# christophmark/bayesloop

Measured on AMD Instinct MI355X. Metric: grid-cells*timesteps/sec (fit()), higher is better.
Workload: dtype f64; 1 GPU; C4 HyperStudy 512x512 grid x 512 sigma values, T=256, full fit (forward+backward+average posterior); T=256, n_hyper=512, mode=full, parallelism=hyper-grid points dealt round-robin to 1 GPU(s), one RCCL gather + one reduce

## Files before the change

bayesloop_amd/csrc/blhip_chainres.hpp:

```cpp
#pragma once
#include "blhip_mfma.hpp"
#include "blhip_resident.hpp"

namespace blc {

using blf::exp_mn;
using blf::reflect1;
using blf::sldi;
using blf::DMAX;
using blk::NRED;
using blm::d4;

constexpr int NT = 512, NW = 8;
constexpr int TM = 16;
constexpr int WCOL = 16;
constexpr int NSLOT = 8;
constexpr int MAXLAG = 4;
constexpr int MAX_STRIPS = 64;
constexpr int SCALE_WAVE = 6;

struct ChainParams {
    int n0, n1, strips;
    int n0t, n1t;
    int T, d, rec_len, lag;
// ... 133 lines not shown
    Q.n0t = own_sgpr(P.n0t);
    Q.n1t = own_sgpr(P.n1t);
    Q.T = own_sgpr(P.T);
    Q.d = own_sgpr(P.d);
    Q.rec_len = own_sgpr(P.rec_len);
    Q.lag = own_sgpr(P.lag);
    Q.means = own_sgpr(P.means);
    Q.strip_major = own_sgpr(P.strip_major);
    Q.B = own_sgpr(P.B);
    Q.nslots = own_sgpr(P.nslots);
    Q.nblk = own_sgpr(P.nblk);
    Q.chain_ids = own_sgpr(P.chain_ids);
    Q.tap_id = own_sgpr(P.tap_id);
    Q.taps = own_sgpr(P.taps);
    Q.tap_off = own_sgpr(P.tap_off);
    Q.tap_lw = own_sgpr(P.tap_lw);
    Q.src0 = own_sgpr(P.src0);
    Q.kinds = own_sgpr(P.kinds);
    Q.reset = own_sgpr(P.reset);
    Q.post = own_sgpr(P.post);
    Q.post_stride = own_sgpr(P.post_stride);
    Q.m0 = own_sgpr(P.m0);
    Q.m1 = own_sgpr(P.m1);
    Q.colA = own_sgpr(P.colA);
    Q.colB = own_sgpr(P.colB);
    Q.rec = own_sgpr(P.rec);
    Q.step0 = own_sgpr(P.step0);
    Q.psum = own_sgpr(P.psum);
    Q.gran = own_sgpr(P.gran);
    Q.sfwd = own_sgpr(P.sfwd);
    Q.wchain = own_sgpr(P.wchain);
    Q.infirst = own_sgpr(P.infirst);
    Q.part = own_sgpr(P.part);
    Q.part_stride = own_sgpr(P.part_stride);
    Q.zeros = own_sgpr(P.zeros);
    Q.part_fresh = own_sgpr(P.part_fresh);
    Q.tshare = own_sgpr(P.tshare);
    Q.bprov = own_sgpr(P.bprov);
    Q.skip_prefix = own_sgpr(P.skip_prefix);
    Q.abort_word = own_sgpr(P.abort_word);
    Q.timeout_ticks = own_sgpr(P.timeout_ticks);
    Q.prof = own_sgpr(P.prof);
    Q.lik = own_sgpr(P.lik);
    Q.tap_id1 = own_sgpr(P.tap_id1);
    Q.xch = own_sgpr(P.xch);
    Q.xch_chain = own_sgpr(P.xch_chain);
    Q.lik_nat = own_sgpr(P.lik_nat);
    Q.xch_mode = own_sgpr(P.xch_mode);
    Q.anch = own_sgpr(P.anch);
    return Q;
}

__device__ __forceinline__ double ldnt(const double *base, unsigned byteoff) { return __builtin_nontemporal_load((const double *)((const char *)base + byteoff)); }
__device__ __forceinline__ void stnt(double *base, unsigned byteoff, double v) { __builtin_nontemporal_store(v, (double *)((char *)base + byteoff)); }

__device__ __forceinline__ double nan_if(bool nan, double x) {
    return __hiloint2double(nan ? 0x7ff80000 : __double2hiint(x), __double2loint(x));
}

#ifndef BLC_BAND4
#define BLC_BAND4 1
#endif
#ifndef BLC_FASTEDGE
#define BLC_FASTEDGE 1
#endif
#ifndef BLC_HOIST_A
#define BLC_HOIST_A 1
#endif
#ifndef BLC_OWNREG
#define BLC_OWNREG 1
#endif
#ifndef BLC_CIRC_RING
#define BLC_CIRC_RING 1
#endif
#ifndef BLC_HOIST_LOOP
#define BLC_HOIST_LOOP 1
#endif
#ifndef BLC_FOLD_HOIST_MAX
#define BLC_FOLD_HOIST_MAX 20
#endif
#ifndef BLC_FOLD4_HOIST_MAX
#define BLC_FOLD4_HOIST_MAX 14
#endif
typedef const double __attribute__((address_space(3))) *band_cp;
template <int NK, int OFF = 0, int NR = NK, int AST = 64>
__device__ __forceinline__ d4 band_products(band_cp Al, const double (&Bv)[NR]) {
    static_assert(OFF + NK <= NR, "the tile's window lies inside the ring");
#if BLC_BAND4
    double a0 = 0.0, a1 = 0.0, a2 = 0.0, a3 = 0.0;
#pragma unroll
    for (int s = 0; s < NK - 3; ++s) {
        const double A = Al[s * AST];
        a0 = __builtin_amdgcn_mfma_f64_4x4x4f64(A, Bv[OFF + s], a0, 0, 0, 0);
        a1 = __builtin_amdgcn_mfma_f64_4x4x4f64(A, Bv[OFF + s + 1], a1, 0, 0, 0);
        a2 = __builtin_amdgcn_mfma_f64_4x4x4f64(A, Bv[OFF + s + 2], a2, 0, 0, 0);
        a3 = __builtin_amdgcn_mfma_f64_4x4x4f64(A, Bv[OFF + s + 3], a3, 0, 0, 0);
    }
    return d4{a0, a1, a2, a3};
#else
    static_assert(AST == 64, "the 16x16x4 form: one entry per lane");
    d4 acc = {0.0, 0.0, 0.0, 0.0};
#pragma unroll
    for (int kb = 0; kb < NK; ++kb) acc = __builtin_amdgcn_mfma_f64_16x16x4f64(Al[kb * 64], Bv[OFF + kb], acc, 0, 0, 0);
    return acc;
#endif
}
template <int NK, int OFF = 0, int NR = NK>
__device__ __forceinline__ d4 band_products_w(const double (&Aw)[NK > 3 ? NK - 3 : 1], const double (&Bv)[NR]) {
    static_assert(OFF + NK <= NR, "the tile's window lies inside the ring");
    double a0 = 0.0, a1 = 0.0, a2 = 0.0, a3 = 0.0;
#pragma unroll
    for (int s = 0; s < NK - 3; ++s) {
        a0 = __builtin_amdgcn_mfma_f64_4x4x4f64(Aw[s], Bv[OFF + s], a0, 0, 0, 0);
        a1 = __builtin_amdgcn_mfma_f64_4x4x4f64(Aw[s], Bv[OFF + s + 1], a1, 0, 0, 0);
        a2 = __builtin_amdgcn_mfma_f64_4x4x4f64(Aw[s], Bv[OFF + s + 2], a2, 0, 0, 0);
        a3 = __builtin_amdgcn_mfma_f64_4x4x4f64(Aw[s], Bv[OFF + s + 3], a3, 0, 0, 0);
    }
    return d4{a0, a1, a2, a3};
}
template <int NK> constexpr int ring_mod() { return NK % 4 == 0 ? NK : NK + 2; }
template <int NK, int NR>
__device__ __forceinline__ d4 band_products_wc(const double (&Aw)[NK > 3 ? NK - 3 : 1], const double (&Bv)[NR], int first) {
    double a0 = 0.0, a1 = 0.0, a2 = 0.0, a3 = 0.0;
#pragma unroll
    for (int s = 0; s < NK - 3; ++s) {
        a0 = __builtin_amdgcn_mfma_f64_4x4x4f64(Aw[s], Bv[(first + s) % NR], a0, 0, 0, 0);
        a1 = __builtin_amdgcn_mfma_f64_4x4x4f64(Aw[s], Bv[(first + s + 1) % NR], a1, 0, 0, 0);
        a2 = __builtin_amdgcn_mfma_f64_4x4x4f64(Aw[s], Bv[(first + s + 2) % NR], a2, 0, 0, 0);
        a3 = __builtin_amdgcn_mfma_f64_4x4x4f64(Aw[s], Bv[(first + s + 3) % NR], a3, 0, 0, 0);
    }
    return d4{a0, a1, a2, a3};
}
template <int NK, int NR, int AST>
__device__ __forceinline__ d4 band_products_c(band_cp Al, const double (&Bv)[NR], int first) {
    double a0 = 0.0, a1 = 0.0, a2 = 0.0, a3 = 0.0;
#pragma unroll
    for (int s = 0; s < NK - 3; ++s) {
        const double A = Al[s * AST];
        a0 = __builtin_amdgcn_mfma_f64_4x4x4f64(A, Bv[(first + s) % NR], a0, 0, 0, 0);
        a1 = __builtin_amdgcn_mfma_f64_4x4x4f64(A, Bv[(first + s + 1) % NR], a1, 0, 0, 0);
        a2 = __builtin_amdgcn_mfma_f64_4x4x4f64(A, Bv[(first + s + 2) % NR], a2, 0, 0, 0);
        a3 = __builtin_amdgcn_mfma_f64_4x4x4f64(A, Bv[(first + s + 3) % NR], a3, 0, 0, 0);
    }
    return d4{a0, a1, a2, a3};
}
__device__ __forceinline__ int band_distance(int e, int R0) {
#if BLC_BAND4
    return abs(4 * (e >> 6) + ((e & 63) >> 4) - R0 - (e & 3));
#else
    return abs(4 * (e >> 6) + ((e & 63) >> 4) - R0 - (e & 15));
#endif
}
__device__ __forceinline__ int band_distance16(int e, int R0) { return abs(4 * (e >> 4) + ((e & 15) >> 2) - R0 - (e & 3)); }


template <int NR>
__device__ __forceinline__ void ring_fill_first_wave(double (&Bv)[NR], const double *S, int g, int c, int k0, int cnt, int rel0) {
    const double *sm = S + (3 - g) * WCOL + c;
    const double *s0 = S + g * WCOL + c;
#pragma unroll
    for (int q = 0; q < NR; ++q) {
        const int rel = rel0 + 4 * q;
        if (q < cnt) Bv[k0 + q] = rel < 0 ? sm[(-rel - 4) * WCOL] : s0[rel * WCOL];
    }
}
template <int N0, int ROWS_W, int NR>
__device__ __forceinline__ void ring_fill_last_wave(double (&Bv)[NR], const double *S, int g, int c, int k0, int cnt, int rel0, int kmod = 0) {
    constexpr int row0 = N0 - ROWS_W;
    const int relmax = rel0 + 4 * (cnt - 1);
    const double *sm = S + (2 * N0 - 1 - row0 - relmax - g) * WCOL + c;
    const double *s0 = S + (row0 + rel0 + g) * WCOL + c;
#pragma unroll
    for (int q = 0; q < NR; ++q) {
        const int rel = rel0 + 4 * q;
        if (q < cnt) Bv[kmod ? (k0 + q) % kmod : k0 + q] = rel >= ROWS_W ? sm[(relmax - rel) * WCOL] : s0[(rel - rel0) * WCOL];
    }
}

template <int NK, int NTW>
constexpr size_t lds_doubles() { return (size_t)(NTW > 4 ? 1 : 2) * NW * NTW * TM * WCOL + NK * (NTW > 4 ? 16 : 64) + NW * NTW * TM + 2 * NW * 4 * 5 + 2 * NSLOT + 8; }

#ifdef BLC_PROF
#define BLC_STAMP(i) do { if (prof_me && k >= 8 && k < 24) P.prof[(wv ? 256 : 0) + (k - 8) * 16 + (i)] = __builtin_readcyclecounter(); } while (0)
#else
#define BLC_STAMP(i) do { } while (0)
#endif

template <int NK, int NTW, bool BWD, bool STORE, bool PAD = false, bool TAB = false>
__global__ __launch_bounds__(NT, 1) void chain_kernel(const ChainParams P) {
    static_assert(!TAB || NTW <= 4, "tabulated likelihood: geometries of <= 512 rows");
    constexpr int R0 = (4 * NK - TM) / 2;
    constexpr int N0 = NW * NTW * TM;
    constexpr int XSZ = N0 * WCOL;
    static_assert(!(PAD && BWD && !STORE) || NTW > 4, "padded grids of <= 512 rows: the folding backward pass is chain_fold2_kernel's");
    static_assert(!(PAD && BWD && STORE && NTW > 4), "padded grids of 1024 rows: posteriors are folded, never stored");
    const int n0t = PAD ? P.n0t : N0, n1t = PAD ? P.n1t : P.n1;
    static_assert(NK == 4 || (NK >= 6 && R0 % 4 == 0), "band = 16 + 2 R0 columns, R0 a multiple of 4; NK = 4: no stencil");
    constexpr bool FILTER = NK > 4;
    constexpr bool TALL = NTW > 4;
    extern __shared__ __attribute__((aligned(16))) double lds[];
    double *const X = lds;
    constexpr int AST = (TALL && BLC_BAND4) ? 16 : 64;
    double *const As = X + (TALL ? 1 : 2) * XSZ;
    double *const m0s = As + NK * AST;
    double *const red = m0s + N0;
    double *const scal = red + 2 * NW * 4 * 5;
    double *const iscal = scal + NSLOT;

    const int tid = threadIdx.x, lane = tid & 63;
    const int wv = __builtin_amdgcn_readfirstlane(tid >> 6);
    const int cs = blockIdx.x / P.strips, tj = blockIdx.x - cs * P.strips;
    const int b = sldi(P.chain_ids, cs);
    const int tap = sldi(P.tap_id, b);
    const int lw0 = tap >= 0 ? sldi(P.tap_lw, tap) : 0;
    const long long o0 = tap >= 0 ? sldi(P.tap_off, tap) : 0;
    const int gj = tj * WCOL + (lane & 15);
    const long long G = (long long)P.n0 * P.n1;
    const int tsh = (!FILTER && P.tshare) ? sldi(P.tshare, b) : 0;

    if (FILTER) for (int e = tid; e < NK * AST; e += NT) As[e] = (AST == 16 ? band_distance16(e, R0) : band_distance(e, R0)) == 0 ? 1.0 : 0.0;
    for (int e = tid; e < N0; e += NT) m0s[e] = P.m0[PAD ? min(e, n0t - 1) : e];
// ... 360 lines not shown
#pragma unroll
                for (int r = 0; r < 4; ++r)
                    al[it % ALD][r] = (it + ALD < NTW) ? ldnt(pstep, cell_off(l, it + ALD, r)) : ldnt(pnext, cell_off(l, it + ALD - NTW, r));
            }
            if ((BWD || STORE) && P.means) {
#pragma unroll
                for (int r = 0; r < 4; ++r) { sM0 = fma(acc[r], m0s[i + g + 4 * r], sM0); sM1 = fma(acc[r], g1, sM1); }
            }

            if (it == 0) BLC_STAMP(4);
            if (it == NTW - 1) BLC_STAMP(5);
            if (FILTER && !WHOLE_RING && it + 1 < NTW) {
#pragma unroll
                for (int kb = 0; kb < NK - 4; ++kb) Bv[kb] = Bv[kb + 4];
                if (FASTEDGE && wv == NW - 1 && (it + 1) * TM + R0 + 12 >= NTW * TM) ring_fill_last_wave<N0, NTW * TM>(Bv, S, g, c, NK - 4, 4, (it + 1) * TM + R0);
                else if (!FASTEDGE && edge) {
#pragma unroll
                    for (int q = 0; q < 4; ++q) Bv[NK - 4 + q] = S[reflect1(i + TM + R0 + 4 * q + g, n0t) * WCOL + c];
                } else {
                    const double *s1 = S + (i + TM + R0 + g) * WCOL + c;
#pragma unroll
                    for (int q = 0; q < 4; ++q) Bv[NK - 4 + q] = s1[q * 4 * WCOL];
                }
            }
        }

        double v[5] = {sN, sS, BWD ? sC : sM0, BWD ? sM0 : sM1, sM1};
        constexpr int NV = BWD ? 5 : 4;
        const int nv = BWD ? (P.means ? 5 : 3) : (P.means ? 4 : ((!FILTER && P.kinds) ? 2 : 1));
        double *rk = red + (k & 1) * (NW * 4 * 5);
#pragma unroll
        for (int q = 0; q < NV; ++q) {
            if (q < nv) {
                double x = v[q];
                x = blk::dpp_add<0x111, 0xf>(x);
                x = blk::dpp_add<0x112, 0xf>(x);
                x = blk::dpp_add<0x114, 0xf>(x);
                x = blk::dpp_add<0x118, 0xf>(x);
                if ((lane & 15) == 15) rk[(wv * 4 + (lane >> 4)) * 5 + q] = x;
            }
        }
        BLC_STAMP(6);
        __syncthreads();
        BLC_STAMP(7);
        if (TALL && FILTER) {
            const int l = fresh_lane(), g = l >> 4, c = l & 15;
#pragma unroll
            for (int it = 0; it < NTW; ++it)
#pragma unroll
                for (int r = 0; r < 4; ++r) D[(row0 + it * TM + g + 4 * r) * WCOL + c] = nst[it][r];
        }
        if (FILTER && k == 0) {
            for (int e = tid; e < NK * AST; e += NT) {
                const int a = AST == 16 ? band_distance16(e, R0) : band_distance(e, R0);
                As[e] = a == 0 ? (lw0 > 0 ? P.taps[o0] : 1.0) : (a <= lw0 ? P.taps[o0 + a] : 0.0);
            }
        }
        if (FILTER && (TALL || k == 0)) __syncthreads();
        if (wv == 5 && lane < nv) {
            double tot = 0.0;
#pragma unroll
            for (int w = 0; w < NW * 4; ++w) tot += rk[w * 5 + lane];
            const int slot = BWD ? lane : (lane < 2 ? lane : lane + 1);
            if (lane == 0 || (BWD ? (P.means || lane < 3) : (lane == 1 ? (!FILTER && P.kinds != nullptr) : P.means != 0)))
                P.psum[(((long long)t * P.B + b) * NRED + slot) * P.nblk + tj] = tot;
            if (lane == (BWD ? 2 : 0)) {
                const unsigned long long bits = (unsigned long long)__double_as_longlong(tot);
                const unsigned long long tag = (unsigned long long)(unsigned)(k + 1) << 32;
                unsigned long long *gw = P.gran + ((((long long)(k & (NSLOT - 1)) * P.nslots + cs) * P.strips + tj) << 1);
                blr::st_u64(gw, tag | (bits & 0xffffffffull));
                blr::st_u64(gw + 1, tag | (bits >> 32));
            }
        }
#pragma unroll
        for (int q = 0; q < DMAX; ++q) xd[q] = xn[q];
        if constexpr (ANCT) anc = anc_next;
    }
}


template <int NK, int NTW>
constexpr size_t lds_doubles_fold2() { return (size_t)2 * NW * NTW * TM * WCOL + 2 * NK * (NK > 24 ? 16 : 64) + NW * NTW * TM + 2 * 2 * NW * 4 * 3 + 4 * NSLOT + 8; }

template <int NK, int NTW>
constexpr size_t lds_doubles_fold4() { return (size_t)2 * NW * NTW * TM * WCOL + 2 * NK * 64 + 4 * 2 * NW * 4 * 3 + 8 * NSLOT + 8; }

template <int NK, int NTW>
__device__ __forceinline__ void chain_fold4_body(const ChainParams &P) {
    static_assert(NK >= 6 && NK <= 24 && NTW >= 1 && NTW <= 4, "four chains per block: ring lengths 6 .. 24 on <= 512 rows");
    constexpr int R0 = (4 * NK - TM) / 2;
    static_assert(R0 % 4 == 0, "band = 16 + 2 R0 columns, R0 a multiple of 4");
    constexpr int N0 = NW * NTW * TM;
    constexpr int XSZ = N0 * WCOL;
    constexpr int AST = 64;
    constexpr int HC = WCOL / 2;
    constexpr unsigned ROWB = HC * 8u, ROW4B = 4u * ROWB;
    extern __shared__ __attribute__((aligned(16))) double lds[];
    double *const X = lds;
    double *const As = X + 2 * XSZ;
    double *const red = As + 2 * NK * AST;
    double *const scal = red + 4 * 2 * NW * 4 * 3;
    double *const iscal = scal + 4 * NSLOT;

    const int tid = threadIdx.x, lane = tid & 63;
    const int wv = __builtin_amdgcn_readfirstlane(tid >> 6);
    const int cs4 = blockIdx.x / P.strips, tj = blockIdx.x - cs4 * P.strips;
    const int nch = min(4, P.nslots - 4 * cs4);
    const int npair = (nch + 1) >> 1;
    int bch[4], lw0[4];
    long long o0[4];
#pragma unroll
    for (int q = 0; q < 4; ++q) {
        bch[q] = sldi(P.chain_ids, 4 * cs4 + min(q, nch - 1));
        const int tap = sldi(P.tap_id, bch[q]);
        lw0[q] = tap >= 0 ? sldi(P.tap_lw, tap) : 0;
        o0[q] = tap >= 0 ? sldi(P.tap_off, tap) : 0;
    }
    const int hl = (lane >> 3) & 1;
    const long long G = (long long)P.n0 * P.n1;

    for (int e = tid; e < 2 * NK * AST; e += NT) As[e] = band_distance(e % (NK * AST), R0) == 0 ? 1.0 : 0.0;
    if (tid < 8 * NSLOT) scal[tid] = 1.0;
    for (int e = tid; e < 2 * XSZ; e += NT) {
        const int q = e % XSZ, row = q >> 4, col = tj * HC + (q & 7);
        X[e] = P.src0[(long long)row * P.n1 + col];
    }
    const double cA = P.colA[tj * HC + (lane & 7)];
    const unsigned strip0 = (unsigned)tj * (unsigned)(P.n0 * HC * 8);
    const int row0 = wv * (NTW * TM);
    auto fresh_lane = [&]() { int l = lane; asm volatile("" : "+v"(l)); return l; };
    auto cell_off = [&](int l, int it) { return __umul24(row0 + it * TM + (l >> 4), ROWB) + strip0 + (unsigned)(l & 7) * 8u; };

    const int t_first = P.T - 1;
    double *const pslot = P.part + (long long)cs4 * P.part_stride;
    int slot_l[2];
    const double *post_l[2], *sfwd_l[2];
    double wch[2], inpred[2];
#pragma unroll
    for (int j = 0; j < 2; ++j) {
        const int q = 2 * j + hl;
        const int b = hl ? bch[2 * j + 1] : bch[2 * j];
        slot_l[j] = min(q, nch - 1) * NSLOT;
        post_l[j] = P.post + (long long)b * P.post_stride;
        sfwd_l[j] = P.sfwd + (long long)b * P.T;
        wch[j] = q < nch ? P.wchain[b] : 0.0;
        inpred[j] = P.infirst[b];
    }
    double stt[NTW][4], al[NTW][4], pacc[NTW][4];
    {
        const double *p0 = post_l[0] + (long long)t_first * G;
        const double *a0 = pslot + (long long)t_first * G;
#pragma unroll
        for (int it = 0; it < NTW; ++it)
#pragma unroll
            for (int r = 0; r < 4; ++r) {
                const unsigned off = cell_off(lane, it) + r * ROW4B;
                al[it][r] = blm::ld32(p0, off);
                pacc[it][r] = (P.part_fresh || (r >> 1) != hl) ? blm::ld32(P.zeros, off & 4088u) : blm::ld32(a0, off);
                stt[it][r] = 0.0;
            }
    }
    double sf_next = 1.0;
    if (wv == SCALE_WAVE || wv == 5 || wv == 0 || wv == NW - 1) __builtin_amdgcn_s_setprio(2);
    bool dead = false;
    typedef const double __attribute__((address_space(3))) *lds_cp;
    unsigned long long gq0[4] = {0ull, 0ull, 0ull, 0ull}, gq1[4] = {0ull, 0ull, 0ull, 0ull};
    double Sprev[4] = {1.0, 1.0, 1.0, 1.0};
    double mq = 1.0, iq = 1.0, dn_prev = -1.0;
    int nq = 0;
    double a_mE = 1.0, a_mR = 1.0, a_iE = 1.0, a_iR = 1.0;
    int a_nE = 0, a_nR = 0;
    const int astrips = P.strips >> 1, atj = tj >> 1;
    auto anchor_lane = [&](int l) { return (l & 0x30) | ((tj & 1) << 3) | (l & 7); };
    AnchorEntry anc_next = anchor_load(P.anch, t_first, wv, astrips, atj, anchor_lane(lane));
    int pend_j = -1, pend_k = 0;

    const LoopParams Q = loop_params(P);
    auto totals = [&](int j, int k) {
        const int hh = (lane >> 3) & 1, q = lane & 7, c = 2 * j + hh;
        if (wv == 5 && lane < 16 && q < 3 && c < nch) {
            const double *rk = red + (c * 2 + (k & 1)) * (NW * 4 * 3);
            double tot = 0.0;
#pragma unroll
            for (int w = 0; w < NW * 4; ++w) tot += rk[w * 3 + q];
            const int t = Q.T - 1 - k;
            const int b = hh ? (j ? bch[3] : bch[1]) : (j ? bch[2] : bch[0]);
            Q.psum[(((long long)t * Q.B + b) * NRED + q) * Q.nblk + tj] = tot;
            if (q == 2) {
                const unsigned long long bits = (unsigned long long)__double_as_longlong(tot);
                const unsigned long long tag = (unsigned long long)(unsigned)(k + 1) << 32;
                unsigned long long *gw = Q.gran + ((((long long)(k & (NSLOT - 1)) * Q.nslots + 4 * cs4 + c) * Q.strips + tj) << 1);
                blr::st_u64(gw, tag | (bits & 0xffffffffull));
                blr::st_u64(gw + 1, tag | (bits >> 32));
            }
        }
    };
    __syncthreads();

    const bool scale_wave = wv == SCALE_WAVE;
    const int nsteps = Q.T * npair;
#pragma unroll 1
    for (int cstep = 0; cstep < nsteps; ++cstep) {
        const int k = npair == 2 ? cstep >> 1 : cstep;
        const int j = __builtin_amdgcn_readfirstlane(npair == 2 ? cstep & 1 : 0);
        const int t = Q.T - 1 - k;
        const int tn = (k + 1 < Q.T) ? t - 1 : t;
        const int jn = k + 1;
        double *const pslot_t = pslot + (long long)t * G;
        double *const pslot_tn = pslot + (long long)tn * G;
        double *const Xj = X + j * XSZ;
        const bool need = scale_wave && jn >= Q.lag && jn < Q.T;
        const bool mine = need && lane < Q.strips;
        unsigned long long hq0[2], hq1[2];
#pragma unroll
        for (int hh = 0; hh < 2; ++hh) {
            hq0[hh] = j ? gq0[2 + hh] : gq0[hh]; hq1[hh] = j ? gq1[2 + hh] : gq1[hh];
            if (scale_wave && 2 * j + hh < nch && jn + 1 >= Q.lag && jn + 1 < Q.T && lane < Q.strips) {
                const unsigned long long *gn = Q.gran + ((((long long)((jn + 1 - Q.lag) & (NSLOT - 1)) * Q.nslots + 4 * cs4 + 2 * j + hh) * Q.strips + lane) << 1);
                const unsigned long long n0_ = blr::ld_u64(gn), n1_ = blr::ld_u64(gn + 1);
                if (j) { gq0[2 + hh] = n0_; gq1[2 + hh] = n1_; } else { gq0[hh] = n0_; gq1[hh] = n1_; }
            }
        }
        const bool last_pair = j + 1 == npair;
        const int tnext = last_pair ? tn : t;
        const double sf_now = sf_next;
        sf_next = (last_pair ? sfwd_l[0] : sfwd_l[1])[min(tnext + 1, Q.T - 1)];
        __syncthreads();
        if (pend_j >= 0) {
            double *const Xp = X + pend_j * XSZ;
            const int l = fresh_lane(), g = l >> 4, c = l & 15;
#pragma unroll
            for (int it = 0; it < NTW; ++it)
#pragma unroll
                for (int r = 0; r < 4; ++r) Xp[(row0 + it * TM + g + 4 * r) * WCOL + c] = stt[it][r];
            totals(pend_j, pend_k);
        }
        if (npair == 1 && pend_j >= 0) __syncthreads();
        pend_j = j; pend_k = k;

        constexpr bool FASTEDGE = BLC_FASTEDGE && NTW * TM >= R0;
        const bool edge = row0 < R0 || row0 + NTW * TM + R0 > N0;
        constexpr int NRM = BLC_CIRC_RING ? ring_mod<NK>() : NK;
        double Bv[NRM];
        {
            const int l = fresh_lane(), g = l >> 4, c = l & 15;
            if (FASTEDGE && wv == 0) ring_fill_first_wave(Bv, Xj, g, c, 0, NK, -R0);
            else if (FASTEDGE && wv == NW - 1 && R0 + 12 >= NTW * TM) ring_fill_last_wave<N0, NTW * TM>(Bv, Xj, g, c, 0, NK, -R0);
            else if (!FASTEDGE && edge) {
#pragma unroll
                for (int kb = 0; kb < NK; ++kb) Bv[kb] = Xj[reflect1(row0 - R0 + 4 * kb + g, N0) * WCOL + c];
            } else {
                const double *s0 = Xj + (row0 - R0 + g) * WCOL + c;
#pragma unroll
                for (int kb = 0; kb < NK; ++kb) Bv[kb] = s0[kb * 4 * WCOL];
            }
        }
        double scale = 1.0, wq = 0.0, wfloor = 0.0;
        double mE = 1.0, mR = 1.0, iE = 1.0, iR = 1.0;
        int nE = 0, nR = 0;
        double sN = 0.0, sS = 0.0, sC = 0.0;
        const double *const pnext = (last_pair ? post_l[0] : post_l[1]) + (long long)tnext * G;

        constexpr bool HOISTA = BLC_HOIST_A && BLC_BAND4 && NTW >= 2 && NK <= BLC_FOLD4_HOIST_MAX;
        double Aw[HOISTA ? NK - 3 : 1];
        if constexpr (HOISTA) {
            const int l = fresh_lane();
            const unsigned aoff = (unsigned)l * 8u + (unsigned)(j * NK * AST * 8);
            lds_cp Al = (lds_cp)((const char __attribute__((address_space(3))) *)(lds_cp)As + aoff);
#pragma unroll
            for (int q = 0; q < NK - 3; ++q) Aw[q] = Al[q * AST];
        }
#pragma unroll
        for (int it = 0; it < NTW; ++it) {
            const int i = row0 + it * TM;
            const int l = fresh_lane(), g = l >> 4, c = l & 15;
            const int h = (l >> 3) & 1;
            d4 acc = {0.0, 0.0, 0.0, 0.0};
            if constexpr (HOISTA) {
                acc = band_products_wc<NK, NRM>(Aw, Bv, BLC_CIRC_RING ? 4 * it : 0);
            } else {
                const unsigned aoff = (unsigned)l * 8u + (unsigned)(j * NK * AST * 8);
                lds_cp Al = (lds_cp)((const char __attribute__((address_space(3))) *)(lds_cp)As + aoff);
                acc = band_products_c<NK, NRM, AST>(Al, Bv, BLC_CIRC_RING ? 4 * it : 0);
            }
            if (it == 0) {
                const int sl = (j ? slot_l[1] : slot_l[0]) + (k & (NSLOT - 1));
                scale = scal[sl];
                double ip = j ? inpred[1] : inpred[0];
                if (k > 0) ip = ip * sf_now * iscal[sl];
                if (j) inpred[1] = ip; else inpred[0] = ip;
                const double wc = j ? wch[1] : wch[0];
                wq = wc * ip; wfloor = wc * 1e-300;
                if (scale_wave) {
#pragma unroll
                    for (int hh = 0; hh < 2; ++hh) {
                        const int cq = 2 * j + hh;
                        if (cq < nch) {
                            double sj = 1.0;
                            if (need) {
                                const unsigned long long *gp = Q.gran + ((((long long)((jn - Q.lag) & (NSLOT - 1)) * Q.nslots + 4 * cs4 + cq) * Q.strips + lane) << 1);
                                const unsigned long long want = (unsigned long long)(unsigned)(jn - Q.lag + 1);
                                unsigned long long q0 = hq0[hh], q1 = hq1[hh];
                                bool ok = !mine || ((q0 >> 32) == want && (q1 >> 32) == want);
                                if (!dead && !__all(ok)) {
                                    const unsigned long long t0 = blr::now_ticks();
                                    for (unsigned spins = 1; !__all(ok); ++spins) {
                                        if (!ok) { q0 = blr::ld_u64(gp); q1 = blr::ld_u64(gp + 1); ok = (q0 >> 32) == want && (q1 >> 32) == want; }
                                        blr::nap();
                                        if ((spins & 255u) == 0u) {
                                            if (blr::ld_flag(Q.abort_word) != 0u) { dead = true; break; }
                                            if (blr::now_ticks() - t0 > Q.timeout_ticks) { blr::st_flag(Q.abort_word, 1u); dead = true; break; }
                                        }
                                    }
                                }
                                const double v = mine ? __longlong_as_double((long long)((q0 & 0xffffffffull) | (q1 << 32))) : 0.0;
                                const double Sg = blk::wave_sum(v);
                                const double sp = j ? Sprev[2 + hh] : Sprev[hh];
                                sj = dead ? 1.0 : sp * scal[cq * NSLOT + ((jn - Q.lag) & (NSLOT - 1))] / Sg;
                                if (j) Sprev[2 + hh] = Sg; else Sprev[hh] = Sg;
                            }
                            if (lane == 0) { scal[cq * NSLOT + (jn & (NSLOT - 1))] = sj; iscal[cq * NSLOT + (jn & (NSLOT - 1))] = 1.0 / sj; }
                        }
                    }
                }
                if (j == 0) {
                    anchor_unpack(anc_next, a_mE, a_nE, a_mR, a_nR);
                    const double dn = anc_next.dn;
                    if (dn != dn_prev) {
                        const double d2 = -32.0 * cA * dn * Q.step0 * Q.step0;
                        int tmp;
                        exp_mn(d2, mq, nq);
                        exp_mn(-d2, iq, tmp);
                        dn_prev = dn;
                    }
                    a_iE = blmath::inv_m(a_mE); a_iR = blmath::inv_m(a_mR);
                    anc_next = anchor_load(Q.anch, tn, wv, astrips, atj, anchor_lane(fresh_lane()));
                }
                mE = a_mE; nE = a_nE; mR = a_mR; nR = a_nR; iE = a_iE; iR = a_iR;
            }

#pragma unroll
            for (int r = 0; r < 4; ++r) {
                const double Lv = ldexp(mE, nE);
                const double beta = acc[r] * scale;
                const double p = al[it][r] * beta;
                const double cn = beta * Lv;
                const double pl = nan_if(Lv == 0.0, ldexp(p * iE, -nE));
                stt[it][r] = cn;
                pacc[it][r] += fmax(p * wq, wfloor);
                sN += p; sS += pl; sC += cn;
                mE *= mR; nE += nR;
                mR *= mq; nR += nq;
                iE *= iR; iR *= iq;
            }
            const unsigned off_t = cell_off(l, it);
            if (last_pair) {
                double tot[4];
#pragma unroll
                for (int r = 0; r < 4; ++r) tot[r] = blk::dpp_add<0x128, 0xf>(pacc[it][r]);
                char *const ps = (char *)pslot_t + off_t + (h ? 2u * ROW4B : 0u);
                __builtin_nontemporal_store(h ? tot[2] : tot[0], (double *)ps);
                __builtin_nontemporal_store(h ? tot[3] : tot[1], (double *)(ps + ROW4B));
                const char *const pz = (const char *)Q.zeros + (off_t & 2040u);
                const char *const pn = (const char *)pslot_tn + off_t;
                const char *const p01 = (Q.part_fresh || h) ? pz : pn, *const p23 = (Q.part_fresh || !h) ? pz : pn;
                pacc[it][0] = __builtin_nontemporal_load((const double *)p01);
                pacc[it][1] = __builtin_nontemporal_load((const double *)(p01 + ROW4B));
                pacc[it][2] = __builtin_nontemporal_load((const double *)(p23 + 2 * ROW4B));
                pacc[it][3] = __builtin_nontemporal_load((const double *)(p23 + 3 * ROW4B));
            }
            {
                const char *const pa_ = (const char *)pnext + off_t;
#pragma unroll
                for (int r = 0; r < 4; ++r) al[it][r] = __builtin_nontemporal_load((const double *)(pa_ + r * ROW4B));
            }
            if (it + 1 < NTW) {
                constexpr bool CIRC = BLC_CIRC_RING != 0;
                if (!CIRC) {
#pragma unroll
                    for (int kb = 0; kb < NK - 4; ++kb) Bv[kb] = Bv[kb + 4];
                }
                const int e0 = CIRC ? 4 * it + NK : NK - 4;
                if (FASTEDGE && wv == NW - 1 && (it + 1) * TM + R0 + 12 >= NTW * TM) ring_fill_last_wave<N0, NTW * TM>(Bv, Xj, g, c, e0, 4, (it + 1) * TM + R0, CIRC ? NRM : 0);
                else if (!FASTEDGE && edge) {
#pragma unroll
                    for (int q = 0; q < 4; ++q) Bv[CIRC ? (e0 + q) % NRM : e0 + q] = Xj[reflect1(i + TM + R0 + 4 * q + g, N0) * WCOL + c];
                } else {
                    const double *s1 = Xj + (i + TM + R0 + g) * WCOL + c;
#pragma unroll
                    for (int q = 0; q < 4; ++q) Bv[CIRC ? (e0 + q) % NRM : e0 + q] = s1[q * 4 * WCOL];
                }
            }
        }

        {
            double v[3] = {sN, sS, sC};
            const int l = fresh_lane();
            double *rk = red + ((2 * j + ((l >> 3) & 1)) * 2 + (k & 1)) * (NW * 4 * 3);
#pragma unroll
            for (int q = 0; q < 3; ++q) {
                double x = v[q];
                x = blk::dpp_add<0x111, 0xf>(x);
                x = blk::dpp_add<0x112, 0xf>(x);
                x = blk::dpp_add<0x114, 0xf>(x);
                if ((l & 7) == 7) rk[(wv * 4 + (l >> 4)) * 3 + q] = x;
            }
        }
        if (k == 0 && last_pair) {
            __syncthreads();
            {
                double *const Xp = X + pend_j * XSZ;
                const int l = fresh_lane(), g = l >> 4, c = l & 15;
#pragma unroll
                for (int it = 0; it < NTW; ++it)
#pragma unroll
                    for (int r = 0; r < 4; ++r) Xp[(row0 + it * TM + g + 4 * r) * WCOL + c] = stt[it][r];
                totals(pend_j, pend_k);
                pend_j = -1;
            }
            for (int e = tid; e < 2 * NK * AST; e += NT) {
                const int jj = e / (NK * AST), q = e - jj * (NK * AST);
                const int cq = 2 * jj + ((q >> 3) & 1);
                const int lw = cq == 0 ? lw0[0] : (cq == 1 ? lw0[1] : (cq == 2 ? lw0[2] : lw0[3]));
                const long long o = cq == 0 ? o0[0] : (cq == 1 ? o0[1] : (cq == 2 ? o0[2] : o0[3]));
                const int a = band_distance(q, R0);
                As[e] = a == 0 ? (lw > 0 ? P.taps[o] : 1.0) : (a <= lw ? P.taps[o + a] : 0.0);
            }
        }
    }
    __syncthreads();
    if (pend_j >= 0) totals(pend_j, pend_k);
}

template <int NK, int NTW, bool PAD, bool QUAD>
__global__ __launch_bounds__(NT, 1) void chain_fold2_kernel(const ChainParams P) {
    static_assert(QUAD && !PAD, "the four-argument flavour: four chains per block on an exact geometry");
    chain_fold4_body<NK, NTW>(P);
}

template <int NK, int NTW, bool PAD = false>
__global__ __launch_bounds__(NT, 1) void chain_fold2_kernel(const ChainParams P) {
    constexpr int R0 = (4 * NK - TM) / 2;
    constexpr int N0 = NW * NTW * TM;
    constexpr int XSZ = N0 * WCOL;
    const int n0t = PAD ? P.n0t : N0, n1t = PAD ? P.n1t : P.n1;
    static_assert(NK == 4 || (NK >= 6 && R0 % 4 == 0), "band = 16 + 2 R0 columns, R0 a multiple of 4; NK = 4: no stencil");
    constexpr bool FILTER = NK > 4;
    extern __shared__ __attribute__((aligned(16))) double lds[];
    double *const X = lds;
    constexpr int AST = (NK > 24 && BLC_BAND4) ? 16 : 64;
    double *const As = X + 2 * XSZ;
    double *const m0s = As + 2 * NK * AST;
    double *const red = m0s + N0;
    double *const scal = red + 2 * 2 * NW * 4 * 3;
    double *const iscal = scal + 2 * NSLOT;

    const int tid = threadIdx.x, lane = tid & 63;
    const int wv = __builtin_amdgcn_readfirstlane(tid >> 6);
    const int cs2 = blockIdx.x / P.strips, tj = blockIdx.x - cs2 * P.strips;
    const int nch = min(2, P.nslots - 2 * cs2);
    int bch[2], tap[2], lw0[2], tshv[2];
    long long o0[2];
#pragma unroll
    for (int j = 0; j < 2; ++j) {
        bch[j] = sldi(P.chain_ids, 2 * cs2 + min(j, nch - 1));
        tshv[j] = P.tshare ? sldi(P.tshare, bch[j]) : 0;
        tap[j] = sldi(P.tap_id, bch[j]);
        lw0[j] = tap[j] >= 0 ? sldi(P.tap_lw, tap[j]) : 0;
        o0[j] = tap[j] >= 0 ? sldi(P.tap_off, tap[j]) : 0;
    }
    const int gj = tj * WCOL + (lane & 15);
    const long long G = (long long)P.n0 * P.n1;

    if (FILTER) for (int e = tid; e < 2 * NK * AST; e += NT) As[e] = (AST == 16 ? band_distance16(e % (NK * AST), R0) : band_distance(e % (NK * AST), R0)) == 0 ? 1.0 : 0.0;
    for (int e = tid; e < N0; e += NT) m0s[e] = P.m0[PAD ? min(e, n0t - 1) : e];
    if (tid < 4 * NSLOT) scal[tid] = 1.0;
    for (int e = tid; e < 2 * XSZ; e += NT) {
        const int q = e % XSZ, row = q >> 4, col = tj * WCOL + (q & 15);
        X[e] = (!PAD || (row < n0t && col < n1t)) ? P.src0[(long long)row * n1t + col] : 0.0;
    }
    const bool colok = !PAD || gj < n1t;
    const int gjc = PAD ? min(gj, n1t - 1) : gj;
    const double cA = P.colA[gjc], cB = P.colB[gjc];
    const unsigned rowx8 = (unsigned)WCOL * 8u;
    const unsigned strip0 = (unsigned)tj * (unsigned)(P.n0 * WCOL * 8);
    const int row0 = wv * (NTW * TM);
    auto fresh_lane = [&]() { int l = lane; asm volatile("" : "+v"(l)); return l; };
    auto cell_off = [&](int l, int it, int r) { return __umul24(row0 + it * TM + (l >> 4) + 4 * r, rowx8) + strip0 + (unsigned)(l & 15) * 8u; };

    const int t_first = P.T - 1;
// ... 311 lines not shown
```

Before: 181.1 billion grid-cells*timesteps/s.

## Defer fold4 state writes past MFMA, partially hoist band A, stage scale tags in LDS

In the four-chain fold kernel, the write of the previous pair's state into LDS is moved from before the MFMA band products to just after the first tile's products. This lets the LDS stores overlap matrix work instead of sitting on the critical path after the barrier. Band matrix entries are now partially hoisted into registers for larger ring lengths, using a per-(NK,NTW) table. Granule tags and the previous scale sums move from per-pair registers into LDS to cut register pressure. The cost is more LDS use, more code paths, and a risk that the reordered state writes race with readers if the barrier assumptions don't hold.

```diff
diff --git a/bayesloop_amd/csrc/blhip_chainres.hpp b/bayesloop_amd/csrc/blhip_chainres.hpp
--- a/bayesloop_amd/csrc/blhip_chainres.hpp
+++ b/bayesloop_amd/csrc/blhip_chainres.hpp
@@ -239,6 +239,15 @@
 #ifndef BLC_FOLD4_HOIST_MAX
 #define BLC_FOLD4_HOIST_MAX 14
 #endif
+#ifndef BLC_FOLD4_LATE_WRITES
+#define BLC_FOLD4_LATE_WRITES 1
+#endif
+#ifndef BLC_FOLD4_SCALE_LDS
+#define BLC_FOLD4_SCALE_LDS 1
+#endif
+#ifndef BLC_FOLD4_HOIST_PART
+#define BLC_FOLD4_HOIST_PART 1
+#endif
 typedef const double __attribute__((address_space(3))) *band_cp;
 template <int NK, int OFF = 0, int NR = NK, int AST = 64>
 __device__ __forceinline__ d4 band_products(band_cp Al, const double (&Bv)[NR]) {
@@ -294,6 +303,20 @@
 #pragma unroll
     for (int s = 0; s < NK - 3; ++s) {
         const double A = Al[s * AST];
+        a0 = __builtin_amdgcn_mfma_f64_4x4x4f64(A, Bv[(first + s) % NR], a0, 0, 0, 0);
+        a1 = __builtin_amdgcn_mfma_f64_4x4x4f64(A, Bv[(first + s + 1) % NR], a1, 0, 0, 0);
+        a2 = __builtin_amdgcn_mfma_f64_4x4x4f64(A, Bv[(first + s + 2) % NR], a2, 0, 0, 0);
+        a3 = __builtin_amdgcn_mfma_f64_4x4x4f64(A, Bv[(first + s + 3) % NR], a3, 0, 0, 0);
+    }
+    return d4{a0, a1, a2, a3};
+}
+template <int NK, int NR, int AST, int H>
+__device__ __forceinline__ d4 band_products_hc(const double (&Aw)[H > 0 ? H : 1], band_cp Al, const double (&Bv)[NR], int first) {
+    static_assert(H >= 0 && H <= NK - 3, "hoisted entries: a prefix of the band");
+    double a0 = 0.0, a1 = 0.0, a2 = 0.0, a3 = 0.0;
+#pragma unroll
+    for (int s = 0; s < NK - 3; ++s) {
+        const double A = s < H ? Aw[s < H ? s : 0] : Al[s * AST];
         a0 = __builtin_amdgcn_mfma_f64_4x4x4f64(A, Bv[(first + s) % NR], a0, 0, 0, 0);
         a1 = __builtin_amdgcn_mfma_f64_4x4x4f64(A, Bv[(first + s + 1) % NR], a1, 0, 0, 0);
         a2 = __builtin_amdgcn_mfma_f64_4x4x4f64(A, Bv[(first + s + 2) % NR], a2, 0, 0, 0);
@@ -820,8 +843,20 @@
 template <int NK, int NTW>
 constexpr size_t lds_doubles_fold2() { return (size_t)2 * NW * NTW * TM * WCOL + 2 * NK * (NK > 24 ? 16 : 64) + NW * NTW * TM + 2 * 2 * NW * 4 * 3 + 4 * NSLOT + 8; }
 
+template <int NK> constexpr bool fold4_scale_lds() { return BLC_FOLD4_SCALE_LDS != 0 && NK <= 20; }
+constexpr int FOLD4_GST = 4 * 64 * 2 + 8;
+template <int NK, int NTW> constexpr int fold4_hoist() {
+    if (!(BLC_HOIST_A && BLC_BAND4) || NTW < 2) return 0;
+    if (NK <= BLC_FOLD4_HOIST_MAX) return NK - 3;
+    if (!BLC_FOLD4_HOIST_PART) return 0;
+    if (NTW == 2) return NK - 3;
+    if (NTW == 3) return NK == 24 ? 15 : NK == 22 ? 17 : NK - 3;
+    return NK == 16 ? 10 : NK == 18 ? 11 : NK == 20 ? 9 : NK == 22 ? 3 : 0;
+}
 template <int NK, int NTW>
-constexpr size_t lds_doubles_fold4() { return (size_t)2 * NW * NTW * TM * WCOL + 2 * NK * 64 + 4 * 2 * NW * 4 * 3 + 8 * NSLOT + 8; }
+constexpr size_t lds_doubles_fold4() {
+    return (size_t)2 * NW * NTW * TM * WCOL + 2 * NK * 64 + 4 * 2 * NW * 4 * 3 + 8 * NSLOT + 8 + (fold4_scale_lds<NK>() ? FOLD4_GST : 0);
+}
 
 template <int NK, int NTW>
 __device__ __forceinline__ void chain_fold4_body(const ChainParams &P) {
@@ -833,12 +868,18 @@
     constexpr int AST = 64;
     constexpr int HC = WCOL / 2;
     constexpr unsigned ROWB = HC * 8u, ROW4B = 4u * ROWB;
+    constexpr int LATE = (NK == 24 && NTW == 4) ? 0 : BLC_FOLD4_LATE_WRITES;
+    static_assert(LATE >= 0 && LATE <= 2, "BLC_FOLD4_LATE_WRITES: 0, 1 or 2");
     extern __shared__ __attribute__((aligned(16))) double lds[];
     double *const X = lds;
     double *const As = X + 2 * XSZ;
     double *const red = As + 2 * NK * AST;
     double *const scal = red + 4 * 2 * NW * 4 * 3;
     double *const iscal = scal + 4 * NSLOT;
+    constexpr bool GLDS = fold4_scale_lds<NK>();
+    static_assert(lds_doubles_fold4<NK, NTW>() * sizeof(double) <= 160 * 1024, "four-chain fold kernel: the LDS of a CU");
+    unsigned long long *const gst = (unsigned long long *)(iscal + 4 * NSLOT + 8);
+    double *const sprv = (double *)(gst + 4 * 64 * 2);
 
     const int tid = threadIdx.x, lane = tid & 63;
     const int wv = __builtin_amdgcn_readfirstlane(tid >> 6);
@@ -859,6 +900,10 @@
 
     for (int e = tid; e < 2 * NK * AST; e += NT) As[e] = band_distance(e % (NK * AST), R0) == 0 ? 1.0 : 0.0;
     if (tid < 8 * NSLOT) scal[tid] = 1.0;
+    if constexpr (GLDS) {
+        for (int e = tid; e < 4 * 64 * 2; e += NT) gst[e] = 0ull;
+        if (tid < 4) sprv[tid] = 1.0;
+    }
     for (int e = tid; e < 2 * XSZ; e += NT) {
         const int q = e % XSZ, row = q >> 4, col = tj * HC + (q & 7);
         X[e] = P.src0[(long long)row * P.n1 + col];
@@ -895,9 +940,16 @@
                 const unsigned off = cell_off(lane, it) + r * ROW4B;
                 al[it][r] = blm::ld32(p0, off);
                 pacc[it][r] = (P.part_fresh || (r >> 1) != hl) ? blm::ld32(P.zeros, off & 4088u) : blm::ld32(a0, off);
-                stt[it][r] = 0.0;
-            }
-    }
+                stt[it][r] = LATE ? P.src0[(long long)(row0 + it * TM + (lane >> 4) + 4 * r) * P.n1 + tj * HC + (lane & 7)] : 0.0;
+            }
+    }
+    auto state_out = [&](double *Xp, int it0, int it1) {
+        const int l = fresh_lane(), g = l >> 4, c = l & 15;
+#pragma unroll
+        for (int it = 0; it < NTW; ++it)
+#pragma unroll
+            for (int r = 0; r < 4; ++r) if (it >= it0 && it < it1) Xp[(row0 + it * TM + g + 4 * r) * WCOL + c] = stt[it][r];
+    };
     double sf_next = 1.0;
     if (wv == SCALE_WAVE || wv == 5 || wv == 0 || wv == NW - 1) __builtin_amdgcn_s_setprio(2);
     bool dead = false;
@@ -913,6 +965,15 @@
     AnchorEntry anc_next = anchor_load(P.anch, t_first, wv, astrips, atj, anchor_lane(lane));
     int pend_j = -1, pend_k = 0;
 
+#ifdef BLC_PROF
+#ifndef BLC_PROF_WAVE4
+#define BLC_PROF_WAVE4 2
+#endif
+    const bool prof_me = blockIdx.x == 0 && lane == 0 && (wv == 0 || wv == BLC_PROF_WAVE4);
+#define BLC_STAMP4(i) do { if (prof_me && cstep >= 16 && cstep < 32) P.prof[(wv ? 256 : 0) + (cstep - 16) * 16 + (i)] = __builtin_readcyclecounter(); } while (0)
+#else
+#define BLC_STAMP4(i) do { } while (0)
+#endif
     const LoopParams Q = loop_params(P);
     auto totals = [&](int j, int k) {
         const int hh = (lane >> 3) & 1, q = lane & 7, c = 2 * j + hh;
@@ -944,19 +1005,34 @@
         const int t = Q.T - 1 - k;
         const int tn = (k + 1 < Q.T) ? t - 1 : t;
         const int jn = k + 1;
+        BLC_STAMP4(0);
         double *const pslot_t = pslot + (long long)t * G;
         double *const pslot_tn = pslot + (long long)tn * G;
         double *const Xj = X + j * XSZ;
         const bool need = scale_wave && jn >= Q.lag && jn < Q.T;
         const bool mine = need && lane < Q.strips;
-        unsigned long long hq0[2], hq1[2];
-#pragma unroll
-        for (int hh = 0; hh < 2; ++hh) {
-            hq0[hh] = j ? gq0[2 + hh] : gq0[hh]; hq1[hh] = j ? gq1[2 + hh] : gq1[hh];
-            if (scale_wave && 2 * j + hh < nch && jn + 1 >= Q.lag && jn + 1 < Q.T && lane < Q.strips) {
-                const unsigned long long *gn = Q.gran + ((((long long)((jn + 1 - Q.lag) & (NSLOT - 1)) * Q.nslots + 4 * cs4 + 2 * j + hh) * Q.strips + lane) << 1);
-                const unsigned long long n0_ = blr::ld_u64(gn), n1_ = blr::ld_u64(gn + 1);
-                if (j) { gq0[2 + hh] = n0_; gq1[2 + hh] = n1_; } else { gq0[hh] = n0_; gq1[hh] = n1_; }
+        [[maybe_unused]] unsigned long long hq0[2], hq1[2];
+        if constexpr (GLDS) {
+            if (scale_wave) {
+                unsigned long long *const gs = gst + ((npair == 2 ? 2 * (1 - j) : 0) * 64 + fresh_lane()) * 2;
+#pragma unroll
+                for (int hh = 0; hh < 2; ++hh) { gs[hh * 128] = gq0[hh]; gs[hh * 128 + 1] = gq1[hh]; }
+            }
+#pragma unroll
+            for (int hh = 0; hh < 2; ++hh)
+                if (scale_wave && 2 * j + hh < nch && jn + 1 >= Q.lag && jn + 1 < Q.T && lane < Q.strips) {
+                    const unsigned long long *gn = Q.gran + ((((long long)((jn + 1 - Q.lag) & (NSLOT - 1)) * Q.nslots + 4 * cs4 + 2 * j + hh) * Q.strips + lane) << 1);
+                    gq0[hh] = blr::ld_u64(gn); gq1[hh] = blr::ld_u64(gn + 1);
+                }
+        } else {
+#pragma unroll
+            for (int hh = 0; hh < 2; ++hh) {
+                hq0[hh] = j ? gq0[2 + hh] : gq0[hh]; hq1[hh] = j ? gq1[2 + hh] : gq1[hh];
+                if (scale_wave && 2 * j + hh < nch && jn + 1 >= Q.lag && jn + 1 < Q.T && lane < Q.strips) {
+                    const unsigned long long *gn = Q.gran + ((((long long)((jn + 1 - Q.lag) & (NSLOT - 1)) * Q.nslots + 4 * cs4 + 2 * j + hh) * Q.strips + lane) << 1);
+                    const unsigned long long n0_ = blr::ld_u64(gn), n1_ = blr::ld_u64(gn + 1);
+                    if (j) { gq0[2 + hh] = n0_; gq1[2 + hh] = n1_; } else { gq0[hh] = n0_; gq1[hh] = n1_; }
+                }
             }
         }
         const bool last_pair = j + 1 == npair;
@@ -964,17 +1040,21 @@
         const double sf_now = sf_next;
         sf_next = (last_pair ? sfwd_l[0] : sfwd_l[1])[min(tnext + 1, Q.T - 1)];
         __syncthreads();
+        BLC_STAMP4(1);
         if (pend_j >= 0) {
-            double *const Xp = X + pend_j * XSZ;
-            const int l = fresh_lane(), g = l >> 4, c = l & 15;
-#pragma unroll
-            for (int it = 0; it < NTW; ++it)
-#pragma unroll
-                for (int r = 0; r < 4; ++r) Xp[(row0 + it * TM + g + 4 * r) * WCOL + c] = stt[it][r];
+            if (!LATE || npair == 1) {
+                double *const Xp = X + pend_j * XSZ;
+                const int l = fresh_lane(), g = l >> 4, c = l & 15;
+#pragma unroll
+                for (int it = 0; it < NTW; ++it)
+#pragma unroll
+                    for (int r = 0; r < 4; ++r) Xp[(row0 + it * TM + g + 4 * r) * WCOL + c] = stt[it][r];
+            }
             totals(pend_j, pend_k);
         }
         if (npair == 1 && pend_j >= 0) __syncthreads();
         pend_j = j; pend_k = k;
+        double *const Xo = X + (1 - j) * XSZ;
 
         constexpr bool FASTEDGE = BLC_FASTEDGE && NTW * TM >= R0;
         const bool edge = row0 < R0 || row0 + NTW * TM + R0 > N0;
@@ -999,29 +1079,34 @@
         double sN = 0.0, sS = 0.0, sC = 0.0;
         const double *const pnext = (last_pair ? post_l[0] : post_l[1]) + (long long)tnext * G;
 
-        constexpr bool HOISTA = BLC_HOIST_A && BLC_BAND4 && NTW >= 2 && NK <= BLC_FOLD4_HOIST_MAX;
-        double Aw[HOISTA ? NK - 3 : 1];
-        if constexpr (HOISTA) {
+        constexpr int H = fold4_hoist<NK, NTW>();
+        double Aw[H > 0 ? H : 1];
+        if constexpr (H > 0) {
             const int l = fresh_lane();
             const unsigned aoff = (unsigned)l * 8u + (unsigned)(j * NK * AST * 8);
             lds_cp Al = (lds_cp)((const char __attribute__((address_space(3))) *)(lds_cp)As + aoff);
 #pragma unroll
-            for (int q = 0; q < NK - 3; ++q) Aw[q] = Al[q * AST];
-        }
+            for (int q = 0; q < H; ++q) Aw[q] = Al[q * AST];
+        }
+        BLC_STAMP4(2);
 #pragma unroll
         for (int it = 0; it < NTW; ++it) {
             const int i = row0 + it * TM;
             const int l = fresh_lane(), g = l >> 4, c = l & 15;
             const int h = (l >> 3) & 1;
             d4 acc = {0.0, 0.0, 0.0, 0.0};
-            if constexpr (HOISTA) {
+            if constexpr (H == NK - 3) {
                 acc = band_products_wc<NK, NRM>(Aw, Bv, BLC_CIRC_RING ? 4 * it : 0);
             } else {
                 const unsigned aoff = (unsigned)l * 8u + (unsigned)(j * NK * AST * 8);
                 lds_cp Al = (lds_cp)((const char __attribute__((address_space(3))) *)(lds_cp)As + aoff);
-                acc = band_products_c<NK, NRM, AST>(Al, Bv, BLC_CIRC_RING ? 4 * it : 0);
-            }
+                if constexpr (H == 0) acc = band_products_c<NK, NRM, AST>(Al, Bv, BLC_CIRC_RING ? 4 * it : 0);
+                else acc = band_products_hc<NK, NRM, AST, H>(Aw, Al, Bv, BLC_CIRC_RING ? 4 * it : 0);
+            }
+            if constexpr (LATE == 1) { if (it == 0) state_out(Xo, 0, NTW); }
+            if constexpr (LATE == 2) state_out(Xo, it, it + 1);
             if (it == 0) {
+                BLC_STAMP4(3);
                 const int sl = (j ? slot_l[1] : slot_l[0]) + (k & (NSLOT - 1));
                 scale = scal[sl];
                 double ip = j ? inpred[1] : inpred[0];
@@ -1038,7 +1123,9 @@
                             if (need) {
                                 const unsigned long long *gp = Q.gran + ((((long long)((jn - Q.lag) & (NSLOT - 1)) * Q.nslots + 4 * cs4 + cq) * Q.strips + lane) << 1);
                                 const unsigned long long want = (unsigned long long)(unsigned)(jn - Q.lag + 1);
-                                unsigned long long q0 = hq0[hh], q1 = hq1[hh];
+                                unsigned long long q0, q1;
+                                if constexpr (GLDS) { const unsigned long long *const gs = gst + (cq * 64 + lane) * 2; q0 = gs[0]; q1 = gs[1]; }
+                                else { q0 = hq0[hh]; q1 = hq1[hh]; }
                                 bool ok = !mine || ((q0 >> 32) == want && (q1 >> 32) == want);
                                 if (!dead && !__all(ok)) {
                                     const unsigned long long t0 = blr::now_ticks();
@@ -1053,9 +1140,11 @@
                                 }
                                 const double v = mine ? __longlong_as_double((long long)((q0 & 0xffffffffull) | (q1 << 32))) : 0.0;
                                 const double Sg = blk::wave_sum(v);
-                                const double sp = j ? Sprev[2 + hh] : Sprev[hh];
+                                double sp;
+                                if constexpr (GLDS) sp = sprv[cq]; else sp = j ? Sprev[2 + hh] : Sprev[hh];
                                 sj = dead ? 1.0 : sp * scal[cq * NSLOT + ((jn - Q.lag) & (NSLOT - 1))] / Sg;
-                                if (j) Sprev[2 + hh] = Sg; else Sprev[hh] = Sg;
+                                if constexpr (GLDS) { if (lane == 0) sprv[cq] = Sg; }
+                                else { if (j) Sprev[2 + hh] = Sg; else Sprev[hh] = Sg; }
                             }
                             if (lane == 0) { scal[cq * NSLOT + (jn & (NSLOT - 1))] = sj; iscal[cq * NSLOT + (jn & (NSLOT - 1))] = 1.0 / sj; }
                         }
@@ -1075,6 +1164,7 @@
                     anc_next = anchor_load(Q.anch, tn, wv, astrips, atj, anchor_lane(fresh_lane()));
                 }
                 mE = a_mE; nE = a_nE; mR = a_mR; nR = a_nR; iE = a_iE; iR = a_iR;
+                BLC_STAMP4(4);
             }
 
 #pragma unroll
@@ -1112,6 +1202,7 @@
 #pragma unroll
                 for (int r = 0; r < 4; ++r) al[it][r] = __builtin_nontemporal_load((const double *)(pa_ + r * ROW4B));
             }
+            if (it == 0) BLC_STAMP4(5);
             if (it + 1 < NTW) {
                 constexpr bool CIRC = BLC_CIRC_RING != 0;
                 if (!CIRC) {
@@ -1131,6 +1222,7 @@
             }
         }
 
+        BLC_STAMP4(6);
         {
             double v[3] = {sN, sS, sC};
             const int l = fresh_lane();
@@ -1144,6 +1236,7 @@
                 if ((l & 7) == 7) rk[(wv * 4 + (l >> 4)) * 3 + q] = x;
             }
         }
+        BLC_STAMP4(7);
         if (k == 0 && last_pair) {
             __syncthreads();
             {
```

Result: no change. 182.8 billion grid-cells*timesteps/s, median of 6 (+0.9%).
